# meilisearch/meilisearch

Measured on NVIDIA H100. Metric: queries/sec (batch=1024, typo-tolerant keyword + 768-d cosine hybrid search, semanticRatio 0.5, top-20), higher is better.
Workload: dtype u64+f16/f32

## Files before the change

meilisearch_b200/csrc/vec_gemm.cu:

```cuda
#include <cuda.h>
#include <cuda_fp16.h>
#include <cuda_runtime.h>

#include <cstdint>
#include <cstdio>
#include <cstdlib>

#include "kernels.h"

namespace b200 {

namespace {

constexpr int GM = VEC_GEMM_QTILE;
constexpr int GN = 64;
constexpr int MN = 2 * GN;
constexpr int GK = 64;
constexpr int STAGES = 4;
constexpr int NACC = 2;
constexpr int ACC_LD = GM + 4;
constexpr int META_BUFS = 2;
constexpr int EPI_WARPS = GM / 32;
constexpr int A_BLOCK = GM * GK * 2;
constexpr int B_BLOCK = MN * GK * 2;
constexpr int ACC_BYTES = GN * ACC_LD * 4;
constexpr int CAND_CAP = VEC_GEMM_CAND_CAP;
constexpr int KMAX = VEC_GEMM_KMAX;
static_assert(GM % 32 == 0 && 2 + EPI_WARPS <= 4, "epilogue warps must fit between warp 1 and the MMA warpgroup");

__device__ __forceinline__ uint32_t smem_u32(const void *p) { return (uint32_t)__cvta_generic_to_shared(p); }

__device__ __forceinline__ void mbar_init(uint64_t *bar, uint32_t count) {
    asm volatile("mbarrier.init.shared::cta.b64 [%0], %1;" ::"r"(smem_u32(bar)), "r"(count));
}
__device__ __forceinline__ void mbar_expect_tx(uint64_t *bar, uint32_t bytes) {
    asm volatile("mbarrier.arrive.expect_tx.shared::cta.b64 _, [%0], %1;" ::"r"(smem_u32(bar)), "r"(bytes) : "memory");
}
__device__ __forceinline__ void mbar_arrive(uint64_t *bar) {
    asm volatile("mbarrier.arrive.shared::cta.b64 _, [%0];" ::"r"(smem_u32(bar)) : "memory");
}
template <int BACKOFF = 0>
__device__ __forceinline__ void mbar_wait(uint64_t *bar, uint32_t parity) {
    uint32_t addr = smem_u32(bar);
    uint32_t done = 0;
    uint64_t spins = 0;
    while (true) {
        asm volatile(
            "{\n\t.reg .pred p;\n\t"
            "mbarrier.try_wait.parity.shared::cta.b64 p, [%1], %2;\n\t"
            "selp.u32 %0, 1, 0, p;\n\t}"
            : "=r"(done)
            : "r"(addr), "r"(parity)
            : "memory");
        if (done) break;
        if (BACKOFF > 0) __nanosleep(BACKOFF);
        if (++spins > (1ull << 26)) __trap();
    }
}
__device__ __forceinline__ void tma_load_2d(void *dst, const CUtensorMap *map, uint64_t *bar, int32_t c0, int32_t c1) {
    asm volatile("cp.async.bulk.tensor.2d.shared::cluster.global.mbarrier::complete_tx::bytes [%0], [%1, {%3, %4}], [%2];" ::"r"(smem_u32(dst)),
                 "l"(reinterpret_cast<uint64_t>(map)), "r"(smem_u32(bar)), "r"(c0), "r"(c1)
                 : "memory");
}
__device__ __forceinline__ bool elect_one() {
    uint32_t pred;
    asm volatile("{\n\t.reg .pred p;\n\telect.sync _|p, 0xffffffff;\n\tselp.u32 %0, 1, 0, p;\n\t}" : "=r"(pred));
    return pred != 0;
}
__device__ __forceinline__ uint64_t make_sdesc(uint32_t saddr) {
    uint64_t d = 0;
    d |= (uint64_t)((saddr & 0x3ffff) >> 4);
    d |= (uint64_t)1 << 16;
    d |= (uint64_t)(1024 >> 4) << 32;
    d |= (uint64_t)1 << 62;
    return d;
}
__device__ __forceinline__ void wgmma_fence() { asm volatile("wgmma.fence.sync.aligned;" ::: "memory"); }
__device__ __forceinline__ void wgmma_commit() { asm volatile("wgmma.commit_group.sync.aligned;" ::: "memory"); }
template <int N>
__device__ __forceinline__ void wgmma_wait() {
    asm volatile("wgmma.wait_group.sync.aligned %0;" ::"n"(N) : "memory");
}
__device__ __forceinline__ void acc_fence(float (&d)[64]) {
#pragma unroll
    for (int i = 0; i < 64; i++) asm volatile("" : "+f"(d[i])::"memory");
}
__device__ __forceinline__ void wgmma_m64n128k16(float (&d)[64], uint64_t adesc, uint64_t bdesc, uint32_t accumulate) {
    asm volatile(
        "{\n\t.reg .pred p;\n\t"
        "setp.ne.b32 p, %66, 0;\n\t"
        "wgmma.mma_async.sync.aligned.m64n128k16.f32.f16.f16 "
        "{%0, %1, %2, %3, %4, %5, %6, %7, %8, %9, %10, %11, %12, %13, %14, %15, "
        "%16, %17, %18, %19, %20, %21, %22, %23, %24, %25, %26, %27, %28, %29, %30, %31, "
        "%32, %33, %34, %35, %36, %37, %38, %39, %40, %41, %42, %43, %44, %45, %46, %47, "
        "%48, %49, %50, %51, %52, %53, %54, %55, %56, %57, %58, %59, %60, %61, %62, %63}, "
        "%64, %65, p, 1, 1, 0, 0;\n\t}"
        : "+f"(d[0]), "+f"(d[1]), "+f"(d[2]), "+f"(d[3]), "+f"(d[4]), "+f"(d[5]), "+f"(d[6]), "+f"(d[7]),
          "+f"(d[8]), "+f"(d[9]), "+f"(d[10]), "+f"(d[11]), "+f"(d[12]), "+f"(d[13]), "+f"(d[14]), "+f"(d[15]),
          "+f"(d[16]), "+f"(d[17]), "+f"(d[18]), "+f"(d[19]), "+f"(d[20]), "+f"(d[21]), "+f"(d[22]), "+f"(d[23]),
          "+f"(d[24]), "+f"(d[25]), "+f"(d[26]), "+f"(d[27]), "+f"(d[28]), "+f"(d[29]), "+f"(d[30]), "+f"(d[31]),
          "+f"(d[32]), "+f"(d[33]), "+f"(d[34]), "+f"(d[35]), "+f"(d[36]), "+f"(d[37]), "+f"(d[38]), "+f"(d[39]),
          "+f"(d[40]), "+f"(d[41]), "+f"(d[42]), "+f"(d[43]), "+f"(d[44]), "+f"(d[45]), "+f"(d[46]), "+f"(d[47]),
          "+f"(d[48]), "+f"(d[49]), "+f"(d[50]), "+f"(d[51]), "+f"(d[52]), "+f"(d[53]), "+f"(d[54]), "+f"(d[55]),
          "+f"(d[56]), "+f"(d[57]), "+f"(d[58]), "+f"(d[59]), "+f"(d[60]), "+f"(d[61]), "+f"(d[62]), "+f"(d[63])
        : "l"(adesc), "l"(bdesc), "r"(accumulate)
        : "memory");
}

__device__ __forceinline__ void cswap(unsigned long long &a, unsigned long long &b, bool asc) {
    unsigned long long lo = a < b ? a : b, hi = a < b ? b : a;
    a = asc ? lo : hi;
    b = asc ? hi : lo;
}
template <int SIZE, int J>
__device__ __forceinline__ void sort_step(unsigned long long (&k)[8], uint32_t lane) {
    if constexpr (J >= 32) {
        constexpr int RJ = J >> 5;
#pragma unroll
        for (int i = 0; i < 8; i++)
            if ((i & RJ) == 0) cswap(k[i], k[i | RJ], ((i * 32) & SIZE) == 0);
    } else {
#pragma unroll
        for (int i = 0; i < 8; i++) {
            const uint32_t e = (uint32_t)i * 32u + lane;
            const unsigned long long o = __shfl_xor_sync(0xffffffffu, k[i], J);
            const bool asc = (e & (uint32_t)SIZE) == 0;
            const bool lower = (lane & (uint32_t)J) == 0;
            const unsigned long long lo = k[i] < o ? k[i] : o, hi = k[i] < o ? o : k[i];
            k[i] = (lower == asc) ? lo : hi;
        }
    }
    if constexpr (J > 1) sort_step<SIZE, J / 2>(k, lane);
}
template <int SIZE>
__device__ __forceinline__ void sort_size(unsigned long long (&k)[8], uint32_t lane) {
    sort_step<SIZE, SIZE / 2>(k, lane);
    if constexpr (SIZE < 256) sort_size<SIZE * 2>(k, lane);
}
__device__ __forceinline__ void warp_sort256(unsigned long long (&k)[8], uint32_t lane) { sort_size<2>(k, lane); }

__device__ __forceinline__ void compact_run(unsigned long long *run, uint32_t c, uint32_t kk, uint32_t kp, uint32_t lane, uint32_t &new_cnt,
                                            unsigned long long &new_thr, unsigned long long &kp_key) {
    unsigned long long k[8];
    __syncwarp();
#pragma unroll
    for (int i = 0; i < 8; i++) {
        uint32_t e = (uint32_t)i * 32u + lane;
        k[i] = e < c ? run[e] : ~0ull;
    }
    warp_sort256(k, lane);
    __syncwarp();
#pragma unroll
    for (int i = 0; i < 8; i++) {
        uint32_t e = (uint32_t)i * 32u + lane;
        if (e < kk) run[e] = k[i];
    }
    const uint32_t ri = (kk - 1) >> 5;
    unsigned long long mine = ri == 0 ? k[0] : (ri == 1 ? k[1] : (ri == 2 ? k[2] : k[3]));
    unsigned long long kth = __shfl_sync(0xffffffffu, mine, (kk - 1) & 31);
    const uint32_t rp = (kp - 1) >> 5;
    unsigned long long minep = rp == 0 ? k[0] : (rp == 1 ? k[1] : (rp == 2 ? k[2] : k[3]));
    unsigned long long kpth = __shfl_sync(0xffffffffu, minep, (kp - 1) & 31);
    new_cnt = c < kk ? c : kk;
    new_thr = c >= kk ? kth : ~0ull;
    kp_key = c >= kp ? kpth : ~0ull;
    __syncwarp();
}

__device__ __forceinline__ float reject_bound(unsigned long long thr, float qn) {
    if (thr == ~0ull || !(qn > 0.f)) return __int_as_float(0xff800000);
    const float dd_thr = __uint_as_float((uint32_t)(thr >> 32));
    const float cs_min = 1.f - 2.f * dd_thr - 4e-7f;
    if (cs_min <= -1.f) return __int_as_float(0xff800000);
    const float x = cs_min / qn;
    return x - fabsf(x) * 2e-6f - 1e-30f;
}

}

__global__ void __launch_bounds__(256, 1)
    vec_gemm_topk_kernel(const __grid_constant__ CUtensorMap tmap_q, const __grid_constant__ CUtensorMap tmap_m, uint64_t n_rows, uint32_t kblocks,
                         uint32_t n_qtiles, uint32_t n_groups, const float *__restrict__ inv_norm, const uint32_t *__restrict__ docids,
                         const float *__restrict__ q_inv_norm, const unsigned long long *__restrict__ cand, uint64_t n_cand_words, uint32_t kk,
                         unsigned long long *__restrict__ gthr ,
                         unsigned long long *__restrict__ runs ,
                         unsigned long long *__restrict__ partial ) {
    extern __shared__ uint8_t smem_raw[];
    uint8_t *smem = reinterpret_cast<uint8_t *>((reinterpret_cast<uintptr_t>(smem_raw) + 1023) & ~(uintptr_t)1023);
    uint8_t *sA = smem;
    uint8_t *sB = sA + (size_t)kblocks * A_BLOCK;
    float *sAcc = reinterpret_cast<float *>(sB + STAGES * B_BLOCK);
    uint64_t *bars = reinterpret_cast<uint64_t *>(sAcc + NACC * (ACC_BYTES / 4));
    uint64_t *a_full = bars, *b_full = bars + 1, *b_empty = b_full + STAGES, *acc_full = b_empty + STAGES, *acc_empty = acc_full + NACC;
    uint64_t *meta_full = acc_empty + NACC, *meta_empty = meta_full + META_BUFS;
    __shared__ __align__(16) uint32_t s_doc[META_BUFS * GN];
    __shared__ __align__(16) float s_scale[META_BUFS * GN];

    const uint32_t warp = threadIdx.x >> 5, lane = threadIdx.x & 31;
    const uint32_t qtile = blockIdx.x % n_qtiles, group = blockIdx.x / n_qtiles;
    if (group >= n_groups) return;
    const uint64_t n_tiles = (n_rows + GN - 1) / GN;
    const uint64_t tile_lo = n_tiles * group / n_groups, tile_hi = n_tiles * (group + 1) / n_groups;

    if (threadIdx.x == 0) {
        mbar_init(a_full, 1);
        for (int s = 0; s < STAGES; s++) {
            mbar_init(b_full + s, 1);
            mbar_init(b_empty + s, 1);
        }
        for (int b = 0; b < NACC; b++) {
            mbar_init(acc_full + b, 128);
            mbar_init(acc_empty + b, EPI_WARPS * 32);
        }
        for (int b = 0; b < META_BUFS; b++) {
            mbar_init(meta_full + b, 1);
            mbar_init(meta_empty + b, EPI_WARPS);
        }
        asm volatile("fence.mbarrier_init.release.cluster;" ::: "memory");
    }
    __syncthreads();

    if (warp == 0) {
        const bool leader = elect_one();
        if (leader) {
            mbar_expect_tx(a_full, kblocks * A_BLOCK);
            for (uint32_t kb = 0; kb < kblocks; kb++) tma_load_2d(sA + (size_t)kb * A_BLOCK, &tmap_q, a_full, (int32_t)(kb * GK), (int32_t)(qtile * GM));
        }
        uint32_t s = 0, ph = 0;
        for (uint64_t t = tile_lo; t < tile_hi; t += 2)
            for (uint32_t kb = 0; kb < kblocks; kb++) {
                mbar_wait<128>(b_empty + s, ph ^ 1);
                if (leader) {
                    mbar_expect_tx(b_full + s, B_BLOCK);
                    tma_load_2d(sB + (size_t)s * B_BLOCK, &tmap_m, b_full + s, (int32_t)(kb * GK), (int32_t)(t * GN));
                }
                __syncwarp();
                if (++s == (uint32_t)STAGES) {
                    s = 0;
                    ph ^= 1;
                }
            }
    } else if (warp == 1) {
        uint32_t n = 0;
        for (uint64_t t = tile_lo; t < tile_hi; t++, n++) {
            const uint32_t mb = n % META_BUFS, mph = (n / META_BUFS) & 1;
            mbar_wait<128>(meta_empty + mb, mph ^ 1);
#pragma unroll
            for (int h = 0; h < GN / 32; h++) {
                const uint64_t r = t * GN + (uint32_t)h * 32u + lane;
                uint32_t doc = 0xffffffffu;
                float sc = 0.f;
                if (r < n_rows) {
                    doc = __ldg(docids + r);
                    sc = __ldg(inv_norm + r);
                    if (!(sc > 0.f)) sc = __int_as_float(0x7f800000);
                    if (cand && !((doc >> 6) < n_cand_words && ((__ldg(cand + (doc >> 6)) >> (doc & 63)) & 1))) doc = 0xffffffffu;
                }
                s_doc[mb * GN + h * 32 + lane] = doc;
                s_scale[mb * GN + h * 32 + lane] = sc;
            }
            __syncwarp();
            if (lane == 0) mbar_arrive(meta_full + mb);
        }
    } else if (warp >= 4) {
        const uint32_t wq = warp - 4, g = lane >> 2, q = lane & 3;
        const uint64_t ad0 = make_sdesc(smem_u32(sA)), bd0 = make_sdesc(smem_u32(sB));
        mbar_wait(a_full, 0);
        uint32_t s = 0, ph = 0, n = 0;
        for (uint64_t t = tile_lo; t < tile_hi; t += 2) {
            float acc[64];
#pragma unroll
            for (int i = 0; i < 64; i++) acc[i] = 0.f;
            uint32_t prev = 0;
            for (uint32_t kb = 0; kb < kblocks; kb++) {
                mbar_wait(b_full + s, ph);
                wgmma_fence();
                acc_fence(acc);
                const uint64_t ad = ad0 + (uint64_t)kb * (A_BLOCK >> 4), bd = bd0 + (uint64_t)s * (B_BLOCK >> 4);
#pragma unroll
                for (uint32_t k = 0; k < GK / 16; k++) wgmma_m64n128k16(acc, ad + 2 * k, bd + 2 * k, (kb | k) != 0);
                wgmma_commit();
                acc_fence(acc);
                if (kb > 0) {
                    wgmma_wait<1>();
                    if (threadIdx.x == 128) mbar_arrive(b_empty + prev);
                }
                prev = s;
                if (++s == (uint32_t)STAGES) {
                    s = 0;
                    ph ^= 1;
                }
            }
            wgmma_wait<0>();
            acc_fence(acc);
            if (threadIdx.x == 128) mbar_arrive(b_empty + prev);
#pragma unroll
            for (int h = 0; h < MN / GN; h++, n++) {
                if (t + h >= tile_hi) break;
                const uint32_t buf = n & 1, aph = (n >> 1) & 1;
                mbar_wait(acc_empty + buf, aph ^ 1);
                float *dst = sAcc + buf * (ACC_BYTES / 4) + wq * 16 + g;
#pragma unroll
                for (int i = 0; i < GN / 8; i++) {
                    const uint32_t c = 8 * i + 2 * q;
                    const int a = 4 * (h * (GN / 8) + i);
                    dst[c * ACC_LD] = acc[a];
                    dst[(c + 1) * ACC_LD] = acc[a + 1];
                    dst[c * ACC_LD + 8] = acc[a + 2];
                    dst[(c + 1) * ACC_LD + 8] = acc[a + 3];
                }
                mbar_arrive(acc_full + buf);
            }
        }
    } else if (warp >= 2 && warp < 2 + EPI_WARPS) {
        const uint32_t w = warp - 2;
        const uint32_t qcol = w * 32 + lane;
        const uint32_t qrow = qtile * GM + qcol;
        const float qn = q_inv_norm[qrow];
        unsigned long long *my_run = runs + ((size_t)blockIdx.x * GM + qcol) * CAND_CAP;
        unsigned long long *warp_runs = runs + ((size_t)blockIdx.x * GM + w * 32) * CAND_CAP;
        uint32_t cnt = 0;
        unsigned long long thr = ~0ull;
        float tq = __int_as_float(0xff800000);
        const uint32_t kp = (kk + n_groups - 1) / n_groups;
        constexpr int KP_REG = 8;
        const bool reg_best = kp <= (uint32_t)KP_REG;
        unsigned long long best[KP_REG];
#pragma unroll
        for (int i = 0; i < KP_REG; i++) best[i] = ~0ull;
        unsigned long long published = ~0ull, best_kp = ~0ull;
        uint32_t n = 0;
        for (uint64_t t = tile_lo; t < tile_hi; t++, n++) {
            const uint32_t buf = n % NACC, aph = (n / NACC) & 1;
            mbar_wait(acc_full + buf, aph);
            const float *col = sAcc + buf * (ACC_BYTES / 4) + qcol;
            float v[GN];
#pragma unroll
            for (int j = 0; j < GN; j++) v[j] = col[j * ACC_LD];
            const uint32_t mb = n % META_BUFS, mph = (n / META_BUFS) & 1;
            mbar_wait(meta_full + mb, mph);
            const uint32_t *tdoc = s_doc + mb * GN;
            const float *tscale = s_scale + mb * GN;
            uint32_t m_lo = 0, m_hi = 0;
#pragma unroll
            for (int j = 0; j < 32; j++) {
                m_lo |= (v[j] * tscale[j] < tq) ? 0u : (1u << j);
                m_hi |= (v[j + 32] * tscale[j + 32] < tq) ? 0u : (1u << j);
            }
            uint32_t u_lo = __reduce_or_sync(0xffffffffu, m_lo), u_hi = __reduce_or_sync(0xffffffffu, m_hi);
            while (u_lo | u_hi) {
                const uint32_t j = u_lo ? (uint32_t)__ffs(u_lo) - 1u : 32u + (uint32_t)__ffs(u_hi) - 1u;
                if (u_lo)
                    u_lo &= u_lo - 1;
                else
                    u_hi &= u_hi - 1;
                const uint32_t mm = j < 32 ? m_lo : m_hi;
                if ((mm >> (j & 31)) & 1u) {
                    const float dot = col[j * ACC_LD];
                    const uint32_t doc = tdoc[j];
                    const float pn = tscale[j] * qn;
                    float dd = 0.f;
                    if (pn > 0.f && isfinite(pn)) {
                        float cs = dot * pn;
                        cs = fminf(1.f, fmaxf(-1.f, cs));
                        dd = (1.f - cs) * 0.5f;
                    }
                    const unsigned long long key = ((unsigned long long)__float_as_uint(dd) << 32) | doc;
                    if (doc != 0xffffffffu && key < thr) {
                        my_run[cnt++] = key;
                        if (reg_best && key < best_kp) {
                            unsigned long long x = key;
#pragma unroll
                            for (int i = 0; i < KP_REG; i++) {
                                const unsigned long long lo = x < best[i] ? x : best[i], hi = x < best[i] ? best[i] : x;
                                best[i] = lo;
                                x = hi;
                            }
                            best_kp = best[0];
#pragma unroll
                            for (int i = 1; i < KP_REG; i++) best_kp = (uint32_t)i < kp ? best[i] : best_kp;
                        }
                    }
                }
            }
            mbar_arrive(acc_empty + buf);
            __syncwarp();
            if (lane == 0) mbar_arrive(meta_empty + mb);
            bool changed = false;
            uint32_t need = __ballot_sync(0xffffffffu, cnt > (uint32_t)(CAND_CAP - GN) || (!reg_best && n == 0 && cnt >= kp));
            while (need) {
                uint32_t l = __ffs(need) - 1;
                need &= need - 1;
                uint32_t c = __shfl_sync(0xffffffffu, cnt, l), nc;
                unsigned long long nt, xp;
                compact_run(warp_runs + (size_t)l * CAND_CAP, c, kk, kp, lane, nc, nt, xp);
                if (lane == l) {
                    cnt = nc;
                    if (nt < thr) {
                        thr = nt;
                        changed = true;
                    }
                    if (!reg_best && xp != ~0ull) gthr[(size_t)qrow * n_groups + group] = xp;
                }
            }
            if (reg_best && best_kp < published) {
                published = best_kp;
                __stcg(gthr + (size_t)qrow * n_groups + group, best_kp);
            }
            if (n < 8 || (n < 64 && (n & 3) == 1) || (n & 15) == 1) {
                const unsigned long long *gx = gthr + (size_t)qrow * n_groups;
                unsigned long long bound = 0;
                for (uint32_t g0 = 0; g0 < n_groups; g0 += 6) {
                    unsigned long long x[6];
#pragma unroll
                    for (int i = 0; i < 6; i++) x[i] = g0 + i < n_groups ? __ldcg(gx + g0 + i) : 0ull;
#pragma unroll
                    for (int i = 0; i < 6; i++) bound = x[i] > bound ? x[i] : bound;
                }
                if (bound < thr) {
                    thr = bound;
                    changed = true;
                }
            }
            if (changed) tq = reject_bound(thr, qn);
        }
        __syncwarp();
        for (uint32_t l = 0; l < 32; l++) {
            uint32_t c = __shfl_sync(0xffffffffu, cnt, l);
            unsigned long long *run = warp_runs + (size_t)l * CAND_CAP;
            unsigned long long k[8];
#pragma unroll
            for (int i = 0; i < 8; i++) {
                uint32_t e = (uint32_t)i * 32u + lane;
                k[i] = e < c ? run[e] : ~0ull;
            }
            warp_sort256(k, lane);
            unsigned long long *out = partial + ((size_t)(qtile * GM + w * 32 + l) * n_groups + group) * KMAX;
#pragma unroll
            for (int i = 0; i < KMAX / 32; i++) {
                uint32_t e = (uint32_t)i * 32u + lane;
                out[e] = e < kk ? k[i] : ~0ull;
            }
        }
    }
    __syncthreads();
}

__global__ void vec_prep_queries_kernel(const float *__restrict__ q, uint32_t n_q, uint32_t n_pad, uint32_t d, __half *__restrict__ out,
                                        float *__restrict__ inv) {
    uint32_t w = (blockIdx.x * blockDim.x + threadIdx.x) >> 5, lane = threadIdx.x & 31;
    if (w >= n_pad) return;
    float s = 0.f;
    for (uint32_t i = lane; i < d; i += 32) {
        float x = w < n_q ? q[(size_t)w * d + i] : 0.f;
        out[(size_t)w * d + i] = __float2half_rn(x);
        s = fmaf(x, x, s);
    }
    for (int o = 16; o; o >>= 1) s += __shfl_xor_sync(0xffffffffu, s, o);
    if (lane == 0) {
        float nrm = sqrtf(s);
        inv[w] = nrm > 0.f ? 1.0f / nrm : 0.f;
    }
}

__global__ void __launch_bounds__(KMAX) vec_merge_kernel(const unsigned long long *__restrict__ partial, uint32_t n_groups, uint32_t kk,
                                                          uint32_t *__restrict__ out_ids, float *__restrict__ out_dist, uint32_t *__restrict__ out_n) {
    __shared__ unsigned long long s[2 * KMAX];
    const uint32_t q = blockIdx.x, t = threadIdx.x;
    const unsigned long long *p = partial + (size_t)q * n_groups * KMAX;
    s[t] = p[t];
    for (uint32_t g = 1; g < n_groups; g++) {
        s[2 * KMAX - 1 - t] = p[(size_t)g * KMAX + t];
        __syncthreads();
        {
            unsigned long long a = s[t], b = s[t + KMAX];
            s[t] = a < b ? a : b;
        }
        __syncthreads();
        for (uint32_t j = KMAX / 2; j >= 1; j >>= 1) {
            uint32_t o = t ^ j;
            unsigned long long a = s[t], b = s[o];
            __syncthreads();
            if (o > t) {
                s[t] = a < b ? a : b;
                s[o] = a < b ? b : a;
            }
            __syncthreads();
        }
    }
    __syncthreads();
    unsigned long long key = s[t];
    if (t < kk) {
        out_ids[(size_t)q * kk + t] = (uint32_t)key;
        out_dist[(size_t)q * kk + t] = __uint_as_float((uint32_t)(key >> 32));
    }
    uint32_t valid = __syncthreads_count(t < kk && key != ~0ull);
    if (t == 0) out_n[q] = valid;
}

namespace {
typedef CUresult (*EncodeTiledFn)(CUtensorMap *, CUtensorMapDataType, cuuint32_t, void *, const cuuint64_t *, const cuuint64_t *, const cuuint32_t *,
                                  const cuuint32_t *, CUtensorMapInterleave, CUtensorMapSwizzle, CUtensorMapL2promotion, CUtensorMapFloatOOBfill);
EncodeTiledFn encode_tiled() {
    static EncodeTiledFn fn = [] {
        void *p = nullptr;
        cudaDriverEntryPointQueryResult qres;
        if (cudaGetDriverEntryPoint("cuTensorMapEncodeTiled", &p, cudaEnableDefault, &qres) != cudaSuccess || qres != cudaDriverEntryPointSuccess)
            p = nullptr;
        return reinterpret_cast<EncodeTiledFn>(p);
    }();
    return fn;
}
bool make_map(CUtensorMap *m, const void *base, uint64_t rows, uint32_t d, uint32_t box_rows) {
    EncodeTiledFn f = encode_tiled();
    if (!f) return false;
    cuuint64_t dims[2] = {d, rows};
    cuuint64_t strides[1] = {(cuuint64_t)d * 2};
    cuuint32_t box[2] = {(cuuint32_t)GK, box_rows};
    cuuint32_t estr[2] = {1, 1};
    return f(m, CU_TENSOR_MAP_DATA_TYPE_FLOAT16, 2, const_cast<void *>(base), dims, strides, box, estr, CU_TENSOR_MAP_INTERLEAVE_NONE,
             CU_TENSOR_MAP_SWIZZLE_128B, CU_TENSOR_MAP_L2_PROMOTION_L2_256B, CU_TENSOR_MAP_FLOAT_OOB_FILL_NONE) == CUDA_SUCCESS;
}
}

size_t vec_gemm_smem_bytes(uint32_t d) {
    return (size_t)(d / GK) * A_BLOCK + (size_t)STAGES * B_BLOCK + (size_t)NACC * ACC_BYTES + 256 + 1023;
}

bool vec_gemm_supported(uint32_t d, uint32_t limit) { return d % GK == 0 && d >= GK && d <= 768 && limit >= 1 && limit <= KMAX; }

cudaError_t launch_vec_prep_queries(cudaStream_t s, const float *q, uint32_t n_q, uint32_t n_pad, uint32_t d, void *out_fp16, float *inv) {
    vec_prep_queries_kernel<<<(n_pad * 32 + 255) / 256, 256, 0, s>>>(q, n_q, n_pad, d, reinterpret_cast<__half *>(out_fp16), inv);
    return cudaGetLastError();
}

cudaError_t launch_vec_gemm_topk(cudaStream_t s, uint32_t sm_count, const void *mat_fp16, const float *inv_norm, const uint32_t *docids, uint64_t n_rows,
                                 uint32_t d, const void *q_fp16, const float *q_inv_norm, uint32_t n_qtiles, uint32_t n_groups,
                                 const unsigned long long *cand, uint64_t n_cand_words, uint32_t k, unsigned long long *gthr, unsigned long long *runs,
                                 unsigned long long *partial, uint32_t *out_ids, float *out_dist, uint32_t *out_n, uint32_t n_q) {
    if (!vec_gemm_supported(d, k) || n_qtiles * n_groups > sm_count || n_groups == 0) return cudaErrorInvalidValue;
    CUtensorMap mq, mm;
    if (!make_map(&mq, q_fp16, (uint64_t)n_qtiles * GM, d, GM) || !make_map(&mm, mat_fp16, n_rows, d, MN)) return cudaErrorNotSupported;
    cudaError_t e = cudaMemsetAsync(gthr, 0xff, (size_t)n_qtiles * GM * n_groups * 8, s);
    if (e != cudaSuccess) return e;
    const size_t smem = vec_gemm_smem_bytes(d);
    e = cudaFuncSetAttribute(vec_gemm_topk_kernel, cudaFuncAttributeMaxDynamicSharedMemorySize, (int)smem);
    if (e != cudaSuccess) return e;
    vec_gemm_topk_kernel<<<n_qtiles * n_groups, 256, smem, s>>>(mq, mm, n_rows, d / GK, n_qtiles, n_groups, inv_norm, docids, q_inv_norm, cand,
                                                                n_cand_words, k, gthr, runs, partial);
    e = cudaGetLastError();
    if (e != cudaSuccess) return e;
    vec_merge_kernel<<<n_q, KMAX, 0, s>>>(partial, n_groups, k, out_ids, out_dist, out_n);
    return cudaGetLastError();
}

}
```

Measured before the change: 12410.

## Double-buffer wgmma accumulators to overlap accumulator hand-off with next tile's MMAs

The MMA warpgroup now keeps two 64-float accumulator sets and alternates between them across tile pairs. After issuing the first k-block of the next tile, it stores the previous tile's accumulators to shared memory for the epilogue, so the tensor cores stay busy during the hand-off. The b_empty release logic now carries across tiles instead of draining with a wait<0> at the end of every tile. The cost is 64 more registers per thread, which risks spills. There is also an ordering subtlety: the previous accumulators are read while a wgmma on the other set may still be in flight.

After: 12660 (median of 6 runs). +2.0%, better.

```diff
diff --git a/meilisearch_b200/csrc/vec_gemm.cu b/meilisearch_b200/csrc/vec_gemm.cu
--- a/meilisearch_b200/csrc/vec_gemm.cu
+++ b/meilisearch_b200/csrc/vec_gemm.cu
@@ -265,35 +265,11 @@
     } else if (warp >= 4) {
         const uint32_t wq = warp - 4, g = lane >> 2, q = lane & 3;
         const uint64_t ad0 = make_sdesc(smem_u32(sA)), bd0 = make_sdesc(smem_u32(sB));
+        const uint64_t nblk = (tile_hi - tile_lo + 1) / 2;
         mbar_wait(a_full, 0);
-        uint32_t s = 0, ph = 0, n = 0;
-        for (uint64_t t = tile_lo; t < tile_hi; t += 2) {
-            float acc[64];
-#pragma unroll
-            for (int i = 0; i < 64; i++) acc[i] = 0.f;
-            uint32_t prev = 0;
-            for (uint32_t kb = 0; kb < kblocks; kb++) {
-                mbar_wait(b_full + s, ph);
-                wgmma_fence();
-                acc_fence(acc);
-                const uint64_t ad = ad0 + (uint64_t)kb * (A_BLOCK >> 4), bd = bd0 + (uint64_t)s * (B_BLOCK >> 4);
-#pragma unroll
-                for (uint32_t k = 0; k < GK / 16; k++) wgmma_m64n128k16(acc, ad + 2 * k, bd + 2 * k, (kb | k) != 0);
-                wgmma_commit();
-                acc_fence(acc);
-                if (kb > 0) {
-                    wgmma_wait<1>();
-                    if (threadIdx.x == 128) mbar_arrive(b_empty + prev);
-                }
-                prev = s;
-                if (++s == (uint32_t)STAGES) {
-                    s = 0;
-                    ph ^= 1;
-                }
-            }
-            wgmma_wait<0>();
-            acc_fence(acc);
-            if (threadIdx.x == 128) mbar_arrive(b_empty + prev);
+        uint32_t s = 0, ph = 0, n = 0, prev = 0;
+        bool pending = false;
+        auto hand_off = [&](float(&acc)[64], uint64_t t) {
 #pragma unroll
             for (int h = 0; h < MN / GN; h++, n++) {
                 if (t + h >= tile_hi) break;
@@ -311,6 +287,49 @@
                 }
                 mbar_arrive(acc_full + buf);
             }
+        };
+        auto issue = [&](float(&cur)[64], uint32_t kb) {
+            mbar_wait(b_full + s, ph);
+            wgmma_fence();
+            acc_fence(cur);
+            const uint64_t ad = ad0 + (uint64_t)kb * (A_BLOCK >> 4), bd = bd0 + (uint64_t)s * (B_BLOCK >> 4);
+#pragma unroll
+            for (uint32_t k = 0; k < GK / 16; k++) wgmma_m64n128k16(cur, ad + 2 * k, bd + 2 * k, (kb | k) != 0);
+            wgmma_commit();
+            acc_fence(cur);
+            if (pending) {
+                wgmma_wait<1>();
+                if (threadIdx.x == 128) mbar_arrive(b_empty + prev);
+            }
+            pending = true;
+            prev = s;
+            if (++s == (uint32_t)STAGES) {
+                s = 0;
+                ph ^= 1;
+            }
+        };
+        auto run_block = [&](float(&cur)[64], float(&last)[64], uint64_t j) {
+            issue(cur, 0);
+            if (j > 0) {
+                acc_fence(last);
+                hand_off(last, tile_lo + 2 * (j - 1));
+            }
+            for (uint32_t kb = 1; kb < kblocks; kb++) issue(cur, kb);
+        };
+        float acc0[64], acc1[64];
+        for (uint64_t j = 0; j < nblk; j += 2) {
+            run_block(acc0, acc1, j);
+            if (j + 1 < nblk) run_block(acc1, acc0, j + 1);
+        }
+        wgmma_wait<0>();
+        acc_fence(acc0);
+        acc_fence(acc1);
+        if (pending && threadIdx.x == 128) mbar_arrive(b_empty + prev);
+        if (nblk > 0) {
+            if ((nblk - 1) & 1)
+                hand_off(acc1, tile_lo + 2 * (nblk - 1));
+            else
+                hand_off(acc0, tile_lo + 2 * (nblk - 1));
         }
     } else if (warp >= 2 && warp < 2 + EPI_WARPS) {
         const uint32_t w = warp - 2;
```
